# TinfoilHat0/Defending-Against-Backdoors-with-Robust-Learning-Rate

Hardware: NVIDIA H100
Metric: fl_rounds_per_sec (higher is better)
Workload: dtype bf16

## Files before the change

### defending-against-backdoors-with-robust-learning-rate_b200/ops/csrc/common.cuh

```cuda
#pragma once
#include <cuda_runtime.h>
#include <cuda_bf16.h>
#include <stdint.h>

#include "dropspec.h"
#include "kernels.h"

#define RLR_CUDA_CHECK(expr)                                                                     \
    do {                                                                                         \
        cudaError_t _e = (expr);                                                                 \
        if (_e != cudaSuccess) return _e;                                                        \
    } while (0)

namespace rlr {

constexpr int kWarp = 32;

__device__ __forceinline__ void pdl_wait() { asm volatile("griddepcontrol.wait;" ::: "memory"); }
__device__ __forceinline__ void pdl_trigger() { asm volatile("griddepcontrol.launch_dependents;" ::: "memory"); }

extern int g_pdl;
bool pdl_enabled();

template <typename... KArgs, typename... Args>
// ... 82 lines not shown
    auto stage = [&](int buf) {
#pragma unroll
        for (int q = 0; q < kPerThread; ++q) tile[buf][r0 + (256 / kCols) * q][c] = v[q];
    };
    load(0);
    stage(0);
    __syncthreads();
    T s = T(0);
    for (int k = 0; k < nchunks; ++k) {
        if (k + 1 < nchunks) load(k + 1);
        if (threadIdx.x < kCols) {
            const int rows = nparts - k * kRows < kRows ? nparts - k * kRows : kRows;
            int r = 0;
            if (k == 0) { s = tile[0][0][threadIdx.x]; r = 1; }
#pragma unroll 8
            for (; r < rows; ++r) s += tile[k & 1][r][threadIdx.x];
        }
        if (k + 1 < nchunks) stage((k + 1) & 1);
        __syncthreads();
    }
    if (threadIdx.x < kCols && col < n) out[col] += s;
}

__device__ __forceinline__ unsigned long long gtimer() {
    unsigned long long t;
    asm volatile("mov.u64 %0, %%globaltimer;" : "=l"(t));
    return t;
}

__device__ __forceinline__ float warp_sum(float v) {
#pragma unroll
    for (int o = 16; o > 0; o >>= 1) v += __shfl_xor_sync(0xffffffffu, v, o);
    return v;
}
__device__ __forceinline__ double warp_sum(double v) {
#pragma unroll
    for (int o = 16; o > 0; o >>= 1) v += __shfl_xor_sync(0xffffffffu, v, o);
    return v;
}
__device__ __forceinline__ unsigned long long warp_sum(unsigned long long v) {
#pragma unroll
    for (int o = 16; o > 0; o >>= 1) v += __shfl_xor_sync(0xffffffffu, v, o);
    return v;
}
__device__ __forceinline__ int warp_sum(int v) {
#pragma unroll
// ... 138 lines not shown
struct AugSpec {
    const long long* stream;
    unsigned long long seed;
    long long start;
    int pad, flip;
};
struct AugDraw { int oy, ox, flip; };
__device__ __forceinline__ AugDraw augment_draw(const AugSpec& a, long long pos) {
    const uint4 u = Philox(a.seed)((uint64_t)pos, (uint64_t)*a.stream);
    const uint32_t n = 2u * (uint32_t)a.pad + 1u;
    return {(int)(u.x % n), (int)(u.y % n), a.flip ? (int)(u.z & 1u) : 0};
}

__device__ __forceinline__ uint32_t dropout_keep8(const DropSpec& d, long long q) {
    const Philox ph(d.seed);
    const uint4 u = ph((uint64_t)q, ((uint64_t)(*d.step) << 20) ^ d.stream);
    const uint32_t r[4] = {u.x, u.y, u.z, u.w};
    uint32_t keep = 0;
#pragma unroll
    for (int i = 0; i < 8; ++i) keep |= (uint32_t)(((r[i >> 1] >> (16 * (i & 1))) & 0xffffu) >= d.thr) << i;
    return keep;
}

template <typename T>
inline cudaError_t launch_ordered_sum(T* out, const T* part, int nparts, long long n, cudaStream_t st) {
    if (nparts >= 16 && n <= 2048)
        return launch_kernel(ordered_sum_narrow_kernel<T>, dim3((unsigned)((n + 7) / 8)), dim3(256), (size_t)0, st, out, part, nparts, n);
    if (nparts >= 16)
        return launch_kernel(ordered_sum_cols_kernel<T>, dim3((unsigned)((n + 31) / 32)), dim3(256), (size_t)0, st, out, part, nparts, n);
    long long blocks = (n + 255) / 256;
    if (blocks > 1024) blocks = 1024;
    if (blocks < 1) blocks = 1;
    return launch_kernel(ordered_sum_kernel<T>, dim3((unsigned)blocks), dim3(256), (size_t)0, st, out, part, nparts, n);
}

__device__ __forceinline__ uint32_t pack_bf16x2(float lo, float hi) {
    __nv_bfloat162 v = __floats2bfloat162_rn(lo, hi);
    return *reinterpret_cast<uint32_t*>(&v);
}

}
```

### defending-against-backdoors-with-robust-learning-rate_b200/ops/csrc/gemm.h

```cpp
#pragma once
#include <cuda_runtime.h>
#include <cuda_bf16.h>
#include <stdint.h>

#include "dropspec.h"

namespace rlr {

constexpr int kStatSlots = 16;

struct ConvGemmParams {
    int M, N, num_kb;
    int mode;
    int cblocks;
    int TW, TH, TN;
    int Ho, Wo, NB;
    int tiles_w, tiles_h;
    int ntaps;
    int in_stride;
    int out_stride, out_ph, out_pw, OutH, OutW;
    int8_t dh[9], dw[9];
    int dn[9];
    int b_mn;
    int wtap[9];
// ... 27 lines not shown
void set_conv_occ3(int level);
void set_conv_one_wave(int on);
void set_conv_tma_store(int on);
void set_conv_split_producer(int on);
void set_conv_trace(long long* buf);
long long* conv_trace_buf();
cudaError_t launch_conv_bf16(const void* x, const void* w, void* out, int NB, int planes, int Hin, int Win, int Cin, int Ho, int Wo,
                             int Cout, int ldc, int ntaps, const int* dh, const int* dw, const int* dplane, const float* bias,
                             int relu, int accumulate, float* stats, cudaStream_t st, const int* wtap = nullptr, int w_taps_total = 0,
                             int in_stride = 1, int out_stride = 1, int out_ph = 0, int out_pw = 0);

cudaError_t launch_conv3x3_halo_bf16(const void* x, const void* w, void* out, int NB, int Hin, int Win, int H, int W, int Cout, const float* bias,
                                     int relu, int accumulate, float* stats, int bo_mode, long long* dbg, int num_sms, cudaStream_t st);

cudaError_t launch_conv3x3_halo3_bf16(const void* x, const void* w, void* out, int NB, int H, int W, int Cout, const float* bias, int relu,
                                      int accumulate, int num_sms, cudaStream_t st);

cudaError_t launch_conv_wgrad_bf16(const void* dy, const void* x, float* dW, int NB, int planes, int Hin, int Win, int Cin, int Cin_valid,
                                   int Ho, int Wo, int Cout, int ntaps, const int* dh, const int* dw, const int* dplane, int num_sms,
                                   cudaStream_t st, int in_stride = 1);
cudaError_t launch_conv_wgrad_halo_bf16(const void* dy, const void* x, float* dW, int NB, int H, int W, int Cin_valid, int Cout,
                                        int num_sms, cudaStream_t st);
cudaError_t launch_linear_wgrad_bf16(const void* dy, const void* x, float* dW, int B, int N, int K, int num_sms, cudaStream_t st);

cudaError_t launch_ordered_sum_f32(float* out, const float* part, int nparts, long long n, cudaStream_t st);
cudaError_t launch_ordered_sum_f64(double* out, const double* part, int nparts, long long n, cudaStream_t st);
cudaError_t launch_channel_stats(const __nv_bfloat16* x, long long M, int C, float* stats , int num_sms, cudaStream_t st,
                                 int only_sum = 0, int nslots = 1);
cudaError_t launch_bn_finalize(const float* stats, int slots, float* mean_rstd, float* running_mean, float* running_var, int C,
                               float count, float eps, float momentum, int train, cudaStream_t st);
cudaError_t launch_bn_apply(const __nv_bfloat16* x, const __nv_bfloat16* res, __nv_bfloat16* y, const float* gamma, const float* beta,
                            float* mean_rstd, long long M, int C, int relu, int fin_mode, const float* stats, int slots, float count,
                            float eps, float momentum, float* running_mean, float* running_var, int num_sms, cudaStream_t st);
cudaError_t launch_bn_bwd_reduce(const __nv_bfloat16* dy, const __nv_bfloat16* y, const __nv_bfloat16* x, const float* mean_rstd,
                                 float* dsum , long long M, int C, int relu, int num_sms, cudaStream_t st,
                                 const float* gamma = nullptr, const float* beta = nullptr, int nslots = 1);
cudaError_t launch_bn_bwd_apply(const __nv_bfloat16* dy, const __nv_bfloat16* y, const __nv_bfloat16* x, const float* gamma,
                                const float* mean_rstd, const float* dsum, __nv_bfloat16* dx, __nv_bfloat16* dres, float* dgamma,
                                float* dbeta, long long M, int C, int relu, int num_sms, cudaStream_t st, const float* beta = nullptr, int nslots = 1);
cudaError_t launch_gn_fwd(const __nv_bfloat16* x, const __nv_bfloat16* res, __nv_bfloat16* y, const float* gamma, const float* beta,
                          float* mean_rstd, int B, int HW, int C, int G, float eps, int relu, int num_sms, cudaStream_t st);
cudaError_t launch_gn_bwd(const __nv_bfloat16* dy, const __nv_bfloat16* y, const __nv_bfloat16* x, const float* gamma,
                          const float* mean_rstd, __nv_bfloat16* dx, __nv_bfloat16* dres, float* dgamma, float* dbeta, int B, int HW,
                          int C, int G, int relu, int num_sms, cudaStream_t st);
cudaError_t launch_relu_bwd(__nv_bfloat16* dy, const __nv_bfloat16* y, long long n, int num_sms, cudaStream_t st, float scale = 1.0f);
cudaError_t launch_maxpool2_fwd(const __nv_bfloat16* x, __nv_bfloat16* y, uint8_t* idx, int B, int H, int W, int C, cudaStream_t st,
                                float drop_p = 0.f, uint64_t seed = 0, const long long* step = nullptr, uint64_t stream = 0);
cudaError_t launch_maxpool2_bwd(const __nv_bfloat16* dy, const uint8_t* idx, __nv_bfloat16* dx, int B, int H, int W, int C, cudaStream_t st,
                                float drop_p, uint64_t seed, const long long* step, uint64_t stream, const __nv_bfloat16* zmask);
// ... 24 lines not shown
```

### defending-against-backdoors-with-robust-learning-rate_b200/ops/csrc/gemm_binding.cpp

```cpp
#include <torch/extension.h>
#include <ATen/cuda/CUDAContext.h>
#include <c10/cuda/CUDAGuard.h>
#include <c10/cuda/CUDAStream.h>
#include <c10/cuda/CUDACachingAllocator.h>

#include <vector>

#include "gemm.h"

namespace rlr {
void* scratch_alloc(size_t bytes, cudaStream_t st) {
    return c10::cuda::CUDACachingAllocator::raw_alloc_with_stream(bytes < 256 ? 256 : bytes, st);
}
void scratch_free(void* p) { c10::cuda::CUDACachingAllocator::raw_delete(p); }
}

namespace {
inline cudaStream_t cur_stream() { return c10::cuda::getCurrentCUDAStream().stream(); }
inline int num_sms() { return at::cuda::getCurrentDeviceProperties()->multiProcessorCount; }
inline void check(cudaError_t e, const char* what) { TORCH_CHECK(e == cudaSuccess, what, ": ", cudaGetErrorString(e)); }
template <typename T>
inline T* opt(const c10::optional<at::Tensor>& t) { return t.has_value() && t->defined() ? reinterpret_cast<T*>(t->data_ptr()) : nullptr; }
inline const __nv_bfloat16* bf(const at::Tensor& t) {
    TORCH_CHECK(t.is_cuda() && t.scalar_type() == at::kBFloat16 && t.is_contiguous(), "expected contiguous CUDA bf16 tensor");
// ... 124 lines not shown
    const int NB = x.size(0), Hin = x.size(1), Win = x.size(2), Cin = x.size(3), Ho = dy.size(1), Wo = dy.size(2), Cout = dy.size(3);
    const int T = (int)dh.size();
    TORCH_CHECK(dW.numel() == (int64_t)Cout * T * cin_valid);
    TORCH_CHECK((Cout <= 64 && Cout % 8 == 0) || Cout % 128 == 0, "wgrad: Cout must be <= 64 or a multiple of 128");
    int a[9], b[9], c[9] = {0};
    for (int t = 0; t < T; ++t) { a[t] = (int)dh[t]; b[t] = (int)dw[t]; }
    check(rlr::launch_conv_wgrad_bf16(bf(dy), bf(x), f32(dW), NB, 1, Hin, Win, Cin, (int)cin_valid, Ho, Wo, Cout, T, a, b, c, num_sms(),
                                      cur_stream(), (int)in_stride), "conv_wgrad_bf16_strided");
}
void conv_wgrad_halo_bf16(at::Tensor dy, at::Tensor x, at::Tensor dW, int64_t cin_valid) {
    c10::cuda::CUDAGuard g(x.device());
    TORCH_CHECK(x.dim() == 4 && x.size(3) == 64 && dy.dim() == 4 && dy.size(0) == x.size(0) && dy.size(1) == x.size(1) && dy.size(2) == x.size(2));
    TORCH_CHECK(dW.numel() == dy.size(3) * 9 * cin_valid);
    check(rlr::launch_conv_wgrad_halo_bf16(bf(dy), bf(x), f32(dW), x.size(0), x.size(1), x.size(2), (int)cin_valid, dy.size(3), num_sms(),
                                           cur_stream()), "conv_wgrad_halo_bf16");
}
void linear_wgrad_bf16(at::Tensor dy, at::Tensor x, at::Tensor dW) {
    c10::cuda::CUDAGuard g(x.device());
    const int B = x.size(0), K = x.size(1), N = dy.size(1);
    TORCH_CHECK(dy.size(0) == B && dW.numel() == (int64_t)N * K && ((N <= 64 && N % 8 == 0) || N % 128 == 0));
    check(rlr::launch_linear_wgrad_bf16(bf(dy), bf(x), f32(dW), B, N, K, num_sms(), cur_stream()), "linear_wgrad_bf16");
}

void ordered_sum(at::Tensor out, at::Tensor part) {
    c10::cuda::CUDAGuard g(out.device());
    TORCH_CHECK(out.is_contiguous() && part.is_contiguous() && part.dim() == 2 && part.size(1) == out.numel() &&
                part.scalar_type() == out.scalar_type(), "ordered_sum: out [n], part [nparts][n]");
    const int nparts = (int)part.size(0);
    const long long n = out.numel();
    if (out.scalar_type() == at::kDouble)
        check(rlr::launch_ordered_sum_f64(out.data_ptr<double>(), part.data_ptr<double>(), nparts, n, cur_stream()), "ordered_sum");
    else
        check(rlr::launch_ordered_sum_f32(out.data_ptr<float>(), part.data_ptr<float>(), nparts, n, cur_stream()), "ordered_sum");
}

void channel_stats(at::Tensor x, at::Tensor stats) {
    c10::cuda::CUDAGuard g(x.device());
    const int C = x.size(-1);
    const int nslots = (int)(stats.numel() / (2 * C));
    TORCH_CHECK(nslots >= 1 && stats.numel() == (int64_t)nslots * 2 * C, "stats must be [slots, 2, C]");
    check(rlr::launch_channel_stats(bf(x), x.numel() / C, C, f32(stats), num_sms(), cur_stream(), 0, nslots), "channel_stats");
}
void bias_grad(at::Tensor dy, at::Tensor db) {
    c10::cuda::CUDAGuard g(dy.device());
    const int C = dy.size(-1);
    TORCH_CHECK(db.numel() == C && db.scalar_type() == at::kFloat && dy.is_contiguous(), "bias_grad: db must be fp32 [C]");
    check(rlr::launch_channel_stats(bf(dy), dy.numel() / C, C, f32(db), num_sms(), cur_stream(), 1), "bias_grad");
}
void bn_finalize(at::Tensor stats, at::Tensor mean_rstd, at::Tensor rm, at::Tensor rv, double count, double eps, double momentum, bool train) {
    c10::cuda::CUDAGuard g(stats.device());
    const int C = mean_rstd.size(-1);
    const int slots = (int)(stats.numel() / (2 * C));
    TORCH_CHECK(slots >= 1 && stats.numel() == (int64_t)slots * 2 * C, "stats must be [slots, 2, C]");
    check(rlr::launch_bn_finalize(f32(stats), slots, f32(mean_rstd), (float*)rm.data_ptr(), (float*)rv.data_ptr(), C, (float)count, (float)eps,
                                  (float)momentum, train, cur_stream()), "bn_finalize");
}
// ... 134 lines not shown
                      bool accumulate_dx) {
    c10::cuda::CUDAGuard g(x.device());
    check(rlr::launch_linear_small_bwd(bf(x), bf(dy), bf(w), const_cast<__nv_bfloat16*>(bfo(dx)), (float*)dw.data_ptr(), opt<float>(db),
                                       x.size(0), x.size(1), w.size(0), accumulate_dx, cur_stream()), "linear_small_bwd");
}
void linear_small_fwd2(at::Tensor x, at::Tensor w, c10::optional<at::Tensor> bias, at::Tensor y, bool relu) {
    c10::cuda::CUDAGuard g(x.device());
    check(rlr::launch_linear_small_fwd2(bf(x), bf(w), opt<const float>(bias), bfm(y), x.size(0), x.size(1), w.size(0), relu, cur_stream()), "linear_small_fwd2");
}
void linear_small_bwd2(at::Tensor x, at::Tensor dy, at::Tensor w, c10::optional<at::Tensor> dx, at::Tensor dw, c10::optional<at::Tensor> db,
                       bool accumulate_dx) {
    c10::cuda::CUDAGuard g(x.device());
    check(rlr::launch_linear_small_bwd2(bf(x), bf(dy), bf(w), const_cast<__nv_bfloat16*>(bfo(dx)), (float*)dw.data_ptr(), opt<float>(db),
                                        x.size(0), x.size(1), w.size(0), accumulate_dx, cur_stream()), "linear_small_bwd2");
}
}

void register_gemm_bindings(py::module_& m) {
    m.attr("STAT_SLOTS") = rlr::kStatSlots;
    m.def("set_persistent_conv", [](bool on) { rlr::set_persistent_conv(on ? 1 : 0); });
    m.def("set_pdl", [](bool on) { rlr::set_pdl(on ? 1 : 0); });
    m.def("set_conv_occ3", [](int64_t level) { rlr::set_conv_occ3((int)level); });
    m.def("set_conv_one_wave", [](bool on) { rlr::set_conv_one_wave(on ? 1 : 0); });
    m.def("set_conv_tma_store", [](bool on) { rlr::set_conv_tma_store(on ? 1 : 0); });
    m.def("set_conv_split_producer", [](bool on) { rlr::set_conv_split_producer(on ? 1 : 0); });
    m.def("set_conv_trace", [](c10::optional<at::Tensor> buf) {
        rlr::set_conv_trace(buf.has_value() && buf->defined() ? reinterpret_cast<long long*>(buf->data_ptr<int64_t>()) : nullptr);
    });
    m.def("gemm_bf16", &gemm_bf16, py::arg("A"), py::arg("B"), py::arg("out"), py::arg("bias"), py::arg("relu"), py::arg("accumulate"), py::arg("stats"),
          py::arg("drop_p") = 0.0, py::arg("drop_seed") = 0, py::arg("drop_step") = py::none(), py::arg("drop_stream") = 0);
    m.def("stem_gemm_bf16", &stem_gemm_bf16, py::arg("A"), py::arg("W"), py::arg("out"), py::arg("bias"), py::arg("relu"), py::arg("stats"),
          py::arg("ready_ptr") = 0, py::arg("lo") = 0, py::arg("hi") = 0, py::arg("epoch") = py::none());
    m.def("gemm_splitk_bf16", &gemm_splitk_bf16, py::arg("A"), py::arg("B"), py::arg("out"), py::arg("ws"), py::arg("bias"), py::arg("relu"),
          py::arg("drop_p") = 0.0, py::arg("drop_seed") = 0, py::arg("drop_step") = py::none(), py::arg("drop_stream") = 0);
    m.def("conv_bf16", &conv_bf16);
    m.def("conv_bf16_strided", &conv_bf16_strided);
    m.def("conv_wgrad_bf16_strided", &conv_wgrad_bf16_strided);
    m.def("conv3x3_halo_bf16", &conv3x3_halo_bf16);
    m.def("conv3x3_halo3_bf16", &conv3x3_halo3_bf16);
    m.def("conv_wgrad_bf16", &conv_wgrad_bf16);
    m.def("linear_wgrad_bf16", &linear_wgrad_bf16);
    m.def("conv_wgrad_halo_bf16", &conv_wgrad_halo_bf16);
    m.def("channel_stats", &channel_stats);
    m.def("ordered_sum", &ordered_sum);
    m.def("bias_grad", &bias_grad);
    m.def("bn_finalize", &bn_finalize);
    m.def("bn_apply", &bn_apply);
    m.def("bn_bwd", &bn_bwd);
    m.def("bn_bwd_recompute", &bn_bwd_recompute);
    m.def("gn_fwd", &gn_fwd);
    m.def("gn_bwd", &gn_bwd);
    m.def("relu_bwd", &relu_bwd, py::arg("dy"), py::arg("y"), py::arg("scale") = 1.0);
    m.def("maxpool2_fwd", &maxpool2_fwd, py::arg("x"), py::arg("y"), py::arg("idx"), py::arg("drop_p") = 0.0, py::arg("drop_seed") = 0,
          py::arg("drop_step") = py::none(), py::arg("drop_stream") = 0);
    m.def("maxpool2_bwd", &maxpool2_bwd, py::arg("dy"), py::arg("idx"), py::arg("dx"), py::arg("drop_p") = 0.0, py::arg("drop_seed") = 0,
          py::arg("drop_step") = py::none(), py::arg("drop_stream") = 0, py::arg("relu_out") = py::none());
    m.def("avgpool_fwd", &avgpool_fwd);
    m.def("avgpool_bwd", &avgpool_bwd);
    m.def("dropout_fwd", &dropout_fwd);
    m.def("dropout_bwd", &dropout_bwd);
    m.def("space_to_depth", &space_to_depth);
    m.def("im2col_small", &im2col_small);
    m.def("filter_transpose", &filter_transpose);
    m.def("depth_to_space", &depth_to_space);
    m.def("filter_gather_transpose", &filter_gather_transpose);
    m.def("linear_small_fwd", &linear_small_fwd);
    m.def("linear_small_bwd", &linear_small_bwd);
// ... 4 lines not shown
```

### defending-against-backdoors-with-robust-learning-rate_b200/ops/csrc/norm.cu

```cuda
#include <stdlib.h>

#include "common.cuh"
#include "gemm.h"

namespace rlr {

struct bf8 { float v[8]; };
__device__ __forceinline__ bf8 unpack8(const uint4& u) {
    const __nv_bfloat162* h = reinterpret_cast<const __nv_bfloat162*>(&u);
    bf8 r;
#pragma unroll
    for (int i = 0; i < 4; ++i) { const float2 f = __bfloat1622float2(h[i]); r.v[2 * i] = f.x; r.v[2 * i + 1] = f.y; }
    return r;
}
__device__ __forceinline__ bf8 load8(const __nv_bfloat16* p) { return unpack8(*reinterpret_cast<const uint4*>(p)); }
__device__ __forceinline__ void store8(__nv_bfloat16* p, const bf8& r) {
    uint4 u;
    u.x = pack_bf16x2(r.v[0], r.v[1]); u.y = pack_bf16x2(r.v[2], r.v[3]);
    u.z = pack_bf16x2(r.v[4], r.v[5]); u.w = pack_bf16x2(r.v[6], r.v[7]);
    *reinterpret_cast<uint4*>(p) = u;
}
static inline int rows_grid(long long M, int rows_per_block, int num_sms, int per_sm) {
    long long want = (M + rows_per_block - 1) / rows_per_block;
    long long cap = (long long)num_sms * per_sm;
// ... 55 lines not shown
                    } else if (kRecompute) {
                        dz.x = (xv.x * msc[2 * i] + msh[2 * i]) > 0.f ? dz.x : 0.f;
                        dz.y = (xv.y * msc[2 * i + 1] + msh[2 * i + 1]) > 0.f ? dz.y : 0.f;
                    }
                    a[2 * i] += dz.x; a[2 * i + 1] += dz.y;
                    b[2 * i] += dz.x * (xv.x - mu[2 * i]) * rs[2 * i]; b[2 * i + 1] += dz.y * (xv.y - mu[2 * i + 1]) * rs[2 * i + 1];
                }
            }
        }
    }
    float* mine = sh + (size_t)ry * 2 * C + cg * 8;
#pragma unroll
    for (int i = 0; i < 8; ++i) { mine[i] = a[i]; mine[C + i] = b[i]; }
    __syncthreads();
    const int ncols = out_cols > 0 ? out_cols : 2 * C;
    float* dst = part + (size_t)blockIdx.x * ncols;
    for (int i = threadIdx.x; i < ncols; i += 256) {
        float t = 0.f;
        for (int r = 0; r < rpi; ++r) t += sh[(size_t)r * 2 * C + i];
        dst[i] = t;
    }
}

cudaError_t launch_ordered_sum_f32(float* out, const float* part, int nparts, long long n, cudaStream_t st) {
    return launch_ordered_sum(out, part, nparts, n, st);
}
cudaError_t launch_ordered_sum_f64(double* out, const double* part, int nparts, long long n, cudaStream_t st) {
    return launch_ordered_sum(out, part, nparts, n, st);
}

cudaError_t launch_channel_stats(const __nv_bfloat16* x, long long M, int C, float* stats, int num_sms, cudaStream_t st, int only_sum, int nslots) {
    if (!chan_ok(C) || nslots < 1) return cudaErrorInvalidValue;
    const int rpi = 256 / (C / 8);
    const int grid = rows_grid(M, rpi * 8, num_sms, nslots >= 4 ? 4 : 2), ncols = only_sum ? C : 2 * C;
    Scratch part((size_t)grid * ncols * sizeof(float), st);
    const size_t smem = (size_t)rpi * 2 * C * sizeof(float);
    auto kernel = nslots >= 4 ? channel_reduce_kernel<0, false, 4, 4> : channel_reduce_kernel<0, false, 8, 2>;
    RLR_CUDA_CHECK(launch_kernel(kernel, dim3(grid), dim3(256), smem, st, x, nullptr, nullptr, nullptr, part.as<float>(), M, C, 0, nullptr,
                                 nullptr, only_sum ? C : 0));
    return launch_ordered_sum(stats, part.as<float>(), grid, (long long)ncols, st);
}
cudaError_t launch_bn_bwd_reduce(const __nv_bfloat16* dy, const __nv_bfloat16* y, const __nv_bfloat16* x, const float* mean_rstd,
                                 float* dsum, long long M, int C, int relu, int num_sms, cudaStream_t st, const float* gamma,
                                 const float* beta, int nslots) {
    if (!chan_ok(C) || (relu == 2 && (!gamma || !beta)) || (relu == 1 && !y) || nslots < 1) return cudaErrorInvalidValue;
    const int rpi = 256 / (C / 8);
    const bool three = nslots >= 3;
    const int grid = rows_grid(M, rpi * 8, num_sms, three ? 3 : 2);
    const size_t smem = (size_t)rpi * 2 * C * sizeof(float);
    Scratch part((size_t)grid * 2 * C * sizeof(float), st);
    if (relu == 2)
// ... 750 lines not shown
```

### defending-against-backdoors-with-robust-learning-rate_b200/ops/csrc/wgrad.cu

```cuda
#include <cuda.h>
#include <stdlib.h>

#include "common.cuh"
#include "gemm.h"
#include "wgmma.cuh"

namespace rlr {

using namespace wg;

cudaError_t make_tmap_bf16(CUtensorMap* map, const void* base, int rank, const uint64_t* dims, const uint64_t* strides_bytes,
                           const uint32_t* box, const uint32_t* elem_strides = nullptr);

constexpr int WG_BM = 128, WG_BK = 64;
constexpr int WG_STAGES = 3;
constexpr int WG_A_BYTES = 2 * 64 * WG_BK * 2;
constexpr int WG_THREADS = 256 + 32;
template <int BNW>
struct WgCfg {
    static constexpr int kGroups = BNW / 64;
    static constexpr int kBBytes = kGroups * 64 * WG_BK * 2;
    static constexpr int kStageBytes = WG_A_BYTES + 3 * kBBytes;
    static constexpr int kSmem = WG_STAGES * kStageBytes + 2048;
};

struct WgradParams {
    int mode;
    int num_kb;
    int kb_per_cta;
    int a_groups;
    int ntaps_cta;
    int T;
    int TW, TH, TN, tiles_w, tiles_h;
    int8_t dh[9], dw[9];
    int dn[9];
    int in_stride;
    int ci_tiles;
    int Cout, Cin_valid;
    float* dW;
    float* part;
};

struct __align__(8) WgShared {
    uint64_t full[WG_STAGES];
    uint64_t empty[WG_STAGES];
};

template <int NACC, int BNW>
__device__ __forceinline__ void wgrad_flush(const float (&acc)[NACC / 2], float* dW, float* part, int co, int Cout, int T, int tap0, int ci0,
                                            int Cin_valid, int t) {
    if (part) dW = part + (size_t)blockIdx.z * Cout * T * Cin_valid;
#pragma unroll
    for (int h = 0; h < 2; ++h) {
        const int row = co + 8 * h;
        if (row >= Cout) continue;
#pragma unroll
        for (int j = 0; j < NACC / 8; ++j) {
            const int c = frag_col(t, 4 * j), tap = c / BNW, ci = ci0 + c % BNW;
            float* dst = dW + ((size_t)row * T + tap0 + tap) * Cin_valid + ci;
            const float a = acc[4 * j + 2 * h], b = acc[4 * j + 2 * h + 1];
            if (part) {
                if (ci < Cin_valid) dst[0] = a;
                if (ci + 1 < Cin_valid) dst[1] = b;
            } else if ((Cin_valid & 1) == 0) {
                if (ci < Cin_valid) asm volatile("red.global.add.v2.f32 [%0], {%1, %2};" ::"l"(dst), "f"(a), "f"(b) : "memory");
            } else {
                if (ci < Cin_valid) atomicAdd(dst, a);
                if (ci + 1 < Cin_valid) atomicAdd(dst + 1, b);
            }
        }
    }
}

template <int BNW, int kTaps>
__global__ void __launch_bounds__(WG_THREADS, 1)
umma_wgrad_kernel(const __grid_constant__ CUtensorMap tmA, const __grid_constant__ CUtensorMap tmB, const WgradParams p) {
    using Cfg = WgCfg<BNW>;
    constexpr int WG_BN = BNW, WG_B_BYTES = Cfg::kBBytes, WG_STAGE_BYTES = Cfg::kStageBytes;
    constexpr int NACC = kTaps * BNW;
    extern __shared__ uint8_t smem_raw[];
    uint8_t* smem = reinterpret_cast<uint8_t*>((reinterpret_cast<uintptr_t>(smem_raw) + 1023) & ~uintptr_t(1023));
    WgShared* sh = reinterpret_cast<WgShared*>(smem + WG_STAGES * WG_STAGE_BYTES);
    const int warp = threadIdx.x >> 5, lane = threadIdx.x & 31;
    const int co_tile = blockIdx.x / p.ci_tiles, ci_tile = blockIdx.x - co_tile * p.ci_tiles;
    const int tap0 = blockIdx.y * kTaps;
    const int kb_begin = blockIdx.z * p.kb_per_cta;
    const int kb_end = min(p.num_kb, kb_begin + p.kb_per_cta);
    const int nkb = kb_end - kb_begin;

    if (warp == 8 && lane == 0) {
        prefetch_tmap(&tmA); prefetch_tmap(&tmB);
        for (int s = 0; s < WG_STAGES; ++s) { mbar_init(&sh->full[s], 1); mbar_init(&sh->empty[s], 8); }
        fence_barrier_init();
    }
    __syncthreads();
    pdl_wait();
    pdl_trigger();

    if (warp == 8) {
        if (lane == 0) {
            int stage = 0;
            uint32_t phase = 0;
            const uint32_t bytes = p.a_groups * 8192 + kTaps * WG_B_BYTES;
            for (int i = 0; i < nkb; ++i) {
                const int kb = kb_begin + i;
                mbar_wait(&sh->empty[stage], phase ^ 1);
                uint8_t* sa = smem + stage * WG_STAGE_BYTES;
                uint8_t* sb = sa + WG_A_BYTES;
                mbar_expect_tx(&sh->full[stage], bytes);
                if (p.mode == 1) {
                    const int tw_i = kb % p.tiles_w, th_i = (kb / p.tiles_w) % p.tiles_h, tn_i = kb / (p.tiles_w * p.tiles_h);
                    const int w0 = tw_i * p.TW, h0 = th_i * p.TH, n0 = tn_i * p.TN;
                    for (int g = 0; g < p.a_groups; ++g)
                        tma_load_4d(&tmA, &sh->full[stage], sa + g * 8192, co_tile * WG_BM + g * 64, w0, h0, n0);
                    for (int t = 0; t < kTaps; ++t)
                        for (int g = 0; g < Cfg::kGroups; ++g)
                            tma_load_4d(&tmB, &sh->full[stage], sb + t * WG_B_BYTES + g * 8192, ci_tile * WG_BN + g * 64,
                                        w0 * p.in_stride + p.dw[tap0 + t], h0 * p.in_stride + p.dh[tap0 + t], n0 + p.dn[tap0 + t]);
                } else {
                    for (int g = 0; g < p.a_groups; ++g)
                        tma_load_2d(&tmA, &sh->full[stage], sa + g * 8192, co_tile * WG_BM + g * 64, kb * WG_BK);
                    for (int g = 0; g < Cfg::kGroups; ++g)
                        tma_load_2d(&tmB, &sh->full[stage], sb + g * 8192, ci_tile * WG_BN + g * 64, kb * WG_BK);
                }
                if (++stage == WG_STAGES) { stage = 0; phase ^= 1; }
            }
        }
    } else if (nkb > 0) {
        const int wgi = threadIdx.x >> 7, t = threadIdx.x & 127;
        const bool active = wgi < p.a_groups;
        float acc[NACC / 2];
#pragma unroll
        for (int i = 0; i < NACC / 2; ++i) acc[i] = 0.f;
        int stage = 0, prev = -1;
        uint32_t phase = 0;
        for (int i = 0; i < nkb; ++i) {
            mbar_wait(&sh->full[stage], phase);
            if (active) {
                const uint32_t sa = smem_u32(smem + stage * WG_STAGE_BYTES) + wgi * 8192;
                const uint32_t sb = smem_u32(smem + stage * WG_STAGE_BYTES) + WG_A_BYTES;
                wgmma_fence();
#pragma unroll
                for (int k = 0; k < WG_BK / 16; ++k) {
                    wgmma_bf16<NACC, 1, 1>(acc, smem_desc_sw128(sa + k * 2048, 8192, 1024), smem_desc_sw128(sb + k * 2048, 8192, 1024),
                                           (i > 0 || k > 0) ? 1u : 0u);
                }
                wgmma_commit();
                wgmma_wait<1>();
            }
            if (prev >= 0 && lane == 0) mbar_arrive(&sh->empty[prev]);
            prev = stage;
            if (++stage == WG_STAGES) { stage = 0; phase ^= 1; }
        }
        if (active) {
            wgmma_wait<0>();
            fence_acc(acc);
            wgrad_flush<NACC, BNW>(acc, p.dW, p.part, co_tile * WG_BM + wgi * 64 + frag_row(t, 0), p.Cout, p.T, tap0, ci_tile * WG_BN, p.Cin_valid, t);
        }
    }
}

template <int BNW, int kTaps>
static cudaError_t launch_wg(const CUtensorMap& tmA, const CUtensorMap& tmB, WgradParams& p, int co_tiles, int tap_groups,
                             int num_sms, cudaStream_t st) {
    static bool configured = false;
    if (!configured) {
        RLR_CUDA_CHECK(cudaFuncSetAttribute(umma_wgrad_kernel<BNW, kTaps>, cudaFuncAttributeMaxDynamicSharedMemorySize, WgCfg<BNW>::kSmem));
        configured = true;
    }
    const int base = co_tiles * p.ci_tiles * tap_groups;
    static const int tune_waves = [] { const char* e = getenv("RLR_WG_WAVES"); return e ? atoi(e) : 0; }();
    int waves = base >= num_sms ? (base + num_sms - 1) / num_sms : (tune_waves > 0 ? tune_waves : 1);
    int splits = (waves * num_sms) / base;
    if (splits > p.num_kb) splits = p.num_kb;
    if (splits < 1) splits = 1;
    p.kb_per_cta = (p.num_kb + splits - 1) / splits;
    splits = (p.num_kb + p.kb_per_cta - 1) / p.kb_per_cta;
    dim3 grid(co_tiles * p.ci_tiles, tap_groups, splits);
    if (splits == 1) return launch_kernel(umma_wgrad_kernel<BNW, kTaps>, grid, dim3(WG_THREADS), (size_t)WgCfg<BNW>::kSmem, st, tmA, tmB, p);
    const long long plane = (long long)p.Cout * p.T * p.Cin_valid;
    Scratch part((size_t)splits * plane * sizeof(float), st);
    p.part = part.as<float>();
    RLR_CUDA_CHECK(launch_kernel(umma_wgrad_kernel<BNW, kTaps>, grid, dim3(WG_THREADS), (size_t)WgCfg<BNW>::kSmem, st, tmA, tmB, p));
    return launch_ordered_sum(p.dW, p.part, splits, plane, st);
}

constexpr int WH_STAGES = 3;
constexpr int WH_A_BYTES = 2 * 128 * 128;
constexpr int WH_HALO_BYTES = 18 * 16 * 128;
constexpr int WH_STAGE_BYTES = WH_A_BYTES + WH_HALO_BYTES;
constexpr int WH_SMEM = WH_STAGES * WH_STAGE_BYTES + 2048;

struct WgHaloParams {
    int NB, H, W, tiles_h, tiles_w;
    int num_kb, kb_per_cta;
    int a_groups;
    int Cout, Cin_valid;
    float* dW;
    float* part;
};

__global__ void __launch_bounds__(WG_THREADS, 1)
umma_wgrad_halo_kernel(const __grid_constant__ CUtensorMap tmA, const __grid_constant__ CUtensorMap tmB, const WgHaloParams p) {
    extern __shared__ uint8_t smem_raw[];
    uint8_t* smem = reinterpret_cast<uint8_t*>((reinterpret_cast<uintptr_t>(smem_raw) + 1023) & ~uintptr_t(1023));
    WgShared* sh = reinterpret_cast<WgShared*>(smem + WH_STAGES * WH_STAGE_BYTES);
// ... 87 lines not shown
    splits = (p.num_kb + p.kb_per_cta - 1) / p.kb_per_cta;
    CUtensorMap tmA, tmB;
    {
        const uint64_t d[4] = {(uint64_t)Cout, (uint64_t)W, (uint64_t)H, (uint64_t)NB};
        const uint64_t s[3] = {(uint64_t)Cout * 2, (uint64_t)W * Cout * 2, (uint64_t)H * W * Cout * 2};
        const uint32_t b[4] = {64, 8, 16, 1};
        RLR_CUDA_CHECK(make_tmap_bf16(&tmA, dy, 4, d, s, b));
    }
    {
        const uint64_t d[4] = {64, (uint64_t)W, (uint64_t)H, (uint64_t)NB};
        const uint64_t s[3] = {128, (uint64_t)W * 128, (uint64_t)H * W * 128};
        const uint32_t b[4] = {64, 16, 18, 1};
        RLR_CUDA_CHECK(make_tmap_bf16(&tmB, x, 4, d, s, b));
    }
    if (splits == 1) return launch_kernel(umma_wgrad_halo_kernel, dim3(co_tiles, 3, splits), dim3(WG_THREADS), (size_t)WH_SMEM, st, tmA, tmB, p);
    const long long plane = (long long)Cout * 9 * Cin_valid;
    Scratch part((size_t)splits * plane * sizeof(float), st);
    p.part = part.as<float>();
    RLR_CUDA_CHECK(launch_kernel(umma_wgrad_halo_kernel, dim3(co_tiles, 3, splits), dim3(WG_THREADS), (size_t)WH_SMEM, st, tmA, tmB, p));
    return launch_ordered_sum(dW, p.part, splits, plane, st);
}

static int pow2_ceil_(int x) { int q = 1; while (q < x) q <<= 1; return q; }

cudaError_t launch_conv_wgrad_bf16(const void* dy, const void* x, float* dW, int NB, int planes, int Hin, int Win, int Cin, int Cin_valid,
                                   int Ho, int Wo, int Cout, int ntaps, const int* dh, const int* dw, const int* dplane, int num_sms,
                                   cudaStream_t st, int in_stride) {
    if (Cin % 64 || Cout % 8 || (ntaps != 1 && ntaps != 9)) return cudaErrorInvalidValue;
    if (in_stride < 1 || in_stride > 2 || (in_stride > 1 && planes != 1)) return cudaErrorInvalidValue;
    WgradParams p{};
    p.in_stride = in_stride;
    int TW = pow2_ceil_(Wo); if (TW > 64) TW = 64;
    int TH = pow2_ceil_(Ho); if (TW * TH > 64) TH = 64 / TW;
    const int TN = 64 / (TW * TH);
    p.mode = 1; p.TW = TW; p.TH = TH; p.TN = TN;
    p.tiles_w = (Wo + TW - 1) / TW; p.tiles_h = (Ho + TH - 1) / TH;
    p.num_kb = p.tiles_w * p.tiles_h * ((NB + TN - 1) / TN);
    p.T = ntaps; p.ntaps_cta = ntaps == 9 ? 3 : 1;
    for (int t = 0; t < ntaps; ++t) { p.dh[t] = (int8_t)dh[t]; p.dw[t] = (int8_t)dw[t]; p.dn[t] = dplane[t] * NB; }
    const bool wide = (Cin % 128 == 0) && (Cin_valid == Cin) && ntaps == 1;
    p.ci_tiles = wide ? Cin / 128 : Cin / 64; p.Cout = Cout; p.Cin_valid = Cin_valid; p.dW = dW;
    p.a_groups = Cout > 64 ? 2 : 1;
    const int co_tiles = (Cout + WG_BM - 1) / WG_BM;
    CUtensorMap tmA, tmB;
    {
        const uint64_t d[4] = {(uint64_t)Cout, (uint64_t)Wo, (uint64_t)Ho, (uint64_t)NB};
        const uint64_t s[3] = {(uint64_t)Cout * 2, (uint64_t)Wo * Cout * 2, (uint64_t)Ho * Wo * Cout * 2};
        const uint32_t b[4] = {64, (uint32_t)TW, (uint32_t)TH, (uint32_t)TN};
        RLR_CUDA_CHECK(make_tmap_bf16(&tmA, dy, 4, d, s, b));
    }
    {
        const uint64_t d[4] = {(uint64_t)Cin, (uint64_t)Win, (uint64_t)Hin, (uint64_t)planes * NB};
        const uint64_t s[3] = {(uint64_t)Cin * 2, (uint64_t)Win * Cin * 2, (uint64_t)Hin * Win * Cin * 2};
        const uint32_t b[4] = {64, (uint32_t)TW, (uint32_t)TH, (uint32_t)TN};
        const uint32_t es[4] = {1, (uint32_t)in_stride, (uint32_t)in_stride, 1};
        RLR_CUDA_CHECK(make_tmap_bf16(&tmB, x, 4, d, s, b, in_stride > 1 ? es : nullptr));
    }
    if (wide) return launch_wg<128, 1>(tmA, tmB, p, co_tiles, ntaps, num_sms, st);
    return ntaps == 9 ? launch_wg<64, 3>(tmA, tmB, p, co_tiles, 3, num_sms, st) : launch_wg<64, 1>(tmA, tmB, p, co_tiles, 1, num_sms, st);
}

cudaError_t launch_linear_wgrad_bf16(const void* dy, const void* x, float* dW, int B, int N, int K, int num_sms, cudaStream_t st) {
    if (N % 8 || K % 64) return cudaErrorInvalidValue;
    WgradParams p{};
    p.mode = 0; p.num_kb = (B + WG_BK - 1) / WG_BK; p.T = 1; p.ntaps_cta = 1; p.in_stride = 1;
    const bool wide = K % 128 == 0;
    p.ci_tiles = wide ? K / 128 : K / 64; p.Cout = N; p.Cin_valid = K; p.dW = dW;
    p.a_groups = N > 64 ? 2 : 1;
    const int co_tiles = (N + WG_BM - 1) / WG_BM;
    CUtensorMap tmA, tmB;
    {
        const uint64_t d[2] = {(uint64_t)N, (uint64_t)B}, s[1] = {(uint64_t)N * 2};
        const uint32_t b[2] = {64, WG_BK};
        RLR_CUDA_CHECK(make_tmap_bf16(&tmA, dy, 2, d, s, b));
    }
    {
        const uint64_t d[2] = {(uint64_t)K, (uint64_t)B}, s[1] = {(uint64_t)K * 2};
        const uint32_t b[2] = {64, WG_BK};
        RLR_CUDA_CHECK(make_tmap_bf16(&tmB, x, 2, d, s, b));
    }
    return wide ? launch_wg<128, 1>(tmA, tmB, p, co_tiles, 1, num_sms, st) : launch_wg<64, 1>(tmA, tmB, p, co_tiles, 1, num_sms, st);
// ... 4 lines not shown
```

Before: 0.6959.

## Load shared halo rows once per tap group in conv wgrad and deepen pipeline

Adds a halo-rows path for 3x3 conv weight-gradient: one TMA box covering the widened row tile is loaded per stage, and the three horizontally shifted taps read it through offset smem descriptors instead of three separate tile loads. Stage count now adapts to shared memory capacity (up to 8) rather than being fixed at 3. It also adds a vectorized wide ordered-sum kernel for few-part, many-column reductions of split-K partials. The risks are wgmma descriptor correctness when reading overlapping swizzled windows and extra template instantiations.

New measurement: 0.7093, median of 6. +1.9%, better.

```diff
diff --git a/defending-against-backdoors-with-robust-learning-rate_b200/ops/csrc/common.cuh b/defending-against-backdoors-with-robust-learning-rate_b200/ops/csrc/common.cuh
--- a/defending-against-backdoors-with-robust-learning-rate_b200/ops/csrc/common.cuh
+++ b/defending-against-backdoors-with-robust-learning-rate_b200/ops/csrc/common.cuh
@@ -128,6 +128,37 @@
     if (threadIdx.x < kCols && col < n) out[col] += s;
 }
 
+template <typename T, int V>
+struct alignas(sizeof(T) * V) SumVec { T v[V]; };
+template <typename T, int V>
+__global__ void __launch_bounds__(256) ordered_sum_wide_kernel(T* __restrict__ out, const T* __restrict__ part, int nparts, long long n) {
+    constexpr int kDepth = 8;
+    using Vec = SumVec<T, V>;
+    pdl_wait();
+    pdl_trigger();
+    const long long units = n / V;
+    for (long long u = (long long)blockIdx.x * 256 + threadIdx.x; u < units; u += (long long)gridDim.x * 256) {
+        const T* src = part + u * V;
+        Vec s = *reinterpret_cast<const Vec*>(src);
+        for (int j0 = 1; j0 < nparts; j0 += kDepth) {
+            Vec v[kDepth];
+#pragma unroll
+            for (int q = 0; q < kDepth; ++q)
+                if (j0 + q < nparts) v[q] = *reinterpret_cast<const Vec*>(src + (size_t)(j0 + q) * n);
+#pragma unroll
+            for (int q = 0; q < kDepth; ++q)
+                if (j0 + q < nparts) {
+#pragma unroll
+                    for (int e = 0; e < V; ++e) s.v[e] += v[q].v[e];
+                }
+        }
+        Vec o = *reinterpret_cast<const Vec*>(out + u * V);
+#pragma unroll
+        for (int e = 0; e < V; ++e) o.v[e] += s.v[e];
+        *reinterpret_cast<Vec*>(out + u * V) = o;
+    }
+}
+
 __device__ __forceinline__ unsigned long long gtimer() {
     unsigned long long t;
     asm volatile("mov.u64 %0, %%globaltimer;" : "=l"(t));
@@ -312,12 +343,31 @@
     return keep;
 }
 
-template <typename T>
-inline cudaError_t launch_ordered_sum(T* out, const T* part, int nparts, long long n, cudaStream_t st) {
-    if (nparts >= 16 && n <= 2048)
+enum OrderedSumKernel { kSumParts = 0, kSumCols = 1, kSumNarrow = 2, kSumWide = 3 };
+constexpr int kWideMaxParts = 16;
+constexpr long long kWideMinCols = 16384;
+inline int ordered_sum_kernel_for(int nparts, long long n) {
+    if (nparts <= kWideMaxParts && n >= kWideMinCols) return kSumWide;
+    if (nparts >= 16) return n <= 2048 ? kSumNarrow : kSumCols;
+    return kSumParts;
+}
+
+template <typename T>
+inline cudaError_t launch_ordered_sum(T* out, const T* part, int nparts, long long n, cudaStream_t st, int kernel = -1) {
+    if (kernel < 0) kernel = ordered_sum_kernel_for(nparts, n);
+    if (kernel == kSumNarrow)
         return launch_kernel(ordered_sum_narrow_kernel<T>, dim3((unsigned)((n + 7) / 8)), dim3(256), (size_t)0, st, out, part, nparts, n);
-    if (nparts >= 16)
+    if (kernel == kSumCols)
         return launch_kernel(ordered_sum_cols_kernel<T>, dim3((unsigned)((n + 31) / 32)), dim3(256), (size_t)0, st, out, part, nparts, n);
+    if (kernel == kSumWide) {
+        constexpr int V = 16 / sizeof(T);
+        const bool vec = n % V == 0 && ((reinterpret_cast<uintptr_t>(out) | reinterpret_cast<uintptr_t>(part)) & 15) == 0;
+        long long blocks = ((vec ? n / V : n) + 255) / 256;
+        if (blocks > 65535) blocks = 65535;
+        if (blocks < 1) blocks = 1;
+        return vec ? launch_kernel(ordered_sum_wide_kernel<T, V>, dim3((unsigned)blocks), dim3(256), (size_t)0, st, out, part, nparts, n)
+                   : launch_kernel(ordered_sum_wide_kernel<T, 1>, dim3((unsigned)blocks), dim3(256), (size_t)0, st, out, part, nparts, n);
+    }
     long long blocks = (n + 255) / 256;
     if (blocks > 1024) blocks = 1024;
     if (blocks < 1) blocks = 1;
diff --git a/defending-against-backdoors-with-robust-learning-rate_b200/ops/csrc/gemm.h b/defending-against-backdoors-with-robust-learning-rate_b200/ops/csrc/gemm.h
--- a/defending-against-backdoors-with-robust-learning-rate_b200/ops/csrc/gemm.h
+++ b/defending-against-backdoors-with-robust-learning-rate_b200/ops/csrc/gemm.h
@@ -73,9 +73,11 @@
 cudaError_t launch_conv_wgrad_halo_bf16(const void* dy, const void* x, float* dW, int NB, int H, int W, int Cin_valid, int Cout,
                                         int num_sms, cudaStream_t st);
 cudaError_t launch_linear_wgrad_bf16(const void* dy, const void* x, float* dW, int B, int N, int K, int num_sms, cudaStream_t st);
+void set_wgrad_halo_rows(int on);
+long long wgrad_halo_rows_launches();
 
-cudaError_t launch_ordered_sum_f32(float* out, const float* part, int nparts, long long n, cudaStream_t st);
-cudaError_t launch_ordered_sum_f64(double* out, const double* part, int nparts, long long n, cudaStream_t st);
+cudaError_t launch_ordered_sum_f32(float* out, const float* part, int nparts, long long n, cudaStream_t st, int kernel = -1);
+cudaError_t launch_ordered_sum_f64(double* out, const double* part, int nparts, long long n, cudaStream_t st, int kernel = -1);
 cudaError_t launch_channel_stats(const __nv_bfloat16* x, long long M, int C, float* stats , int num_sms, cudaStream_t st,
                                  int only_sum = 0, int nslots = 1);
 cudaError_t launch_bn_finalize(const float* stats, int slots, float* mean_rstd, float* running_mean, float* running_var, int C,
diff --git a/defending-against-backdoors-with-robust-learning-rate_b200/ops/csrc/gemm_binding.cpp b/defending-against-backdoors-with-robust-learning-rate_b200/ops/csrc/gemm_binding.cpp
--- a/defending-against-backdoors-with-robust-learning-rate_b200/ops/csrc/gemm_binding.cpp
+++ b/defending-against-backdoors-with-robust-learning-rate_b200/ops/csrc/gemm_binding.cpp
@@ -170,16 +170,17 @@
     check(rlr::launch_linear_wgrad_bf16(bf(dy), bf(x), f32(dW), B, N, K, num_sms(), cur_stream()), "linear_wgrad_bf16");
 }
 
-void ordered_sum(at::Tensor out, at::Tensor part) {
+void ordered_sum(at::Tensor out, at::Tensor part, int64_t kernel) {
     c10::cuda::CUDAGuard g(out.device());
     TORCH_CHECK(out.is_contiguous() && part.is_contiguous() && part.dim() == 2 && part.size(1) == out.numel() &&
                 part.scalar_type() == out.scalar_type(), "ordered_sum: out [n], part [nparts][n]");
+    TORCH_CHECK(kernel >= -1 && kernel <= 3, "ordered_sum: kernel must be -1 (rule) or 0..3");
     const int nparts = (int)part.size(0);
     const long long n = out.numel();
     if (out.scalar_type() == at::kDouble)
-        check(rlr::launch_ordered_sum_f64(out.data_ptr<double>(), part.data_ptr<double>(), nparts, n, cur_stream()), "ordered_sum");
+        check(rlr::launch_ordered_sum_f64(out.data_ptr<double>(), part.data_ptr<double>(), nparts, n, cur_stream(), (int)kernel), "ordered_sum");
     else
-        check(rlr::launch_ordered_sum_f32(out.data_ptr<float>(), part.data_ptr<float>(), nparts, n, cur_stream()), "ordered_sum");
+        check(rlr::launch_ordered_sum_f32(out.data_ptr<float>(), part.data_ptr<float>(), nparts, n, cur_stream(), (int)kernel), "ordered_sum");
 }
 
 void channel_stats(at::Tensor x, at::Tensor stats) {
@@ -360,6 +361,8 @@
     m.def("set_pdl", [](bool on) { rlr::set_pdl(on ? 1 : 0); });
     m.def("set_conv_occ3", [](int64_t level) { rlr::set_conv_occ3((int)level); });
     m.def("set_conv_one_wave", [](bool on) { rlr::set_conv_one_wave(on ? 1 : 0); });
+    m.def("set_wgrad_halo_rows", [](bool on) { rlr::set_wgrad_halo_rows(on ? 1 : 0); });
+    m.def("wgrad_halo_rows_launches", []() { return (int64_t)rlr::wgrad_halo_rows_launches(); });
     m.def("set_conv_tma_store", [](bool on) { rlr::set_conv_tma_store(on ? 1 : 0); });
     m.def("set_conv_split_producer", [](bool on) { rlr::set_conv_split_producer(on ? 1 : 0); });
     m.def("set_conv_trace", [](c10::optional<at::Tensor> buf) {
@@ -380,7 +383,7 @@
     m.def("linear_wgrad_bf16", &linear_wgrad_bf16);
     m.def("conv_wgrad_halo_bf16", &conv_wgrad_halo_bf16);
     m.def("channel_stats", &channel_stats);
-    m.def("ordered_sum", &ordered_sum);
+    m.def("ordered_sum", &ordered_sum, py::arg("out"), py::arg("part"), py::arg("kernel") = -1);
     m.def("bias_grad", &bias_grad);
     m.def("bn_finalize", &bn_finalize);
     m.def("bn_apply", &bn_apply);
diff --git a/defending-against-backdoors-with-robust-learning-rate_b200/ops/csrc/norm.cu b/defending-against-backdoors-with-robust-learning-rate_b200/ops/csrc/norm.cu
--- a/defending-against-backdoors-with-robust-learning-rate_b200/ops/csrc/norm.cu
+++ b/defending-against-backdoors-with-robust-learning-rate_b200/ops/csrc/norm.cu
@@ -101,11 +101,11 @@
     }
 }
 
-cudaError_t launch_ordered_sum_f32(float* out, const float* part, int nparts, long long n, cudaStream_t st) {
-    return launch_ordered_sum(out, part, nparts, n, st);
-}
-cudaError_t launch_ordered_sum_f64(double* out, const double* part, int nparts, long long n, cudaStream_t st) {
-    return launch_ordered_sum(out, part, nparts, n, st);
+cudaError_t launch_ordered_sum_f32(float* out, const float* part, int nparts, long long n, cudaStream_t st, int kernel) {
+    return launch_ordered_sum(out, part, nparts, n, st, kernel);
+}
+cudaError_t launch_ordered_sum_f64(double* out, const double* part, int nparts, long long n, cudaStream_t st, int kernel) {
+    return launch_ordered_sum(out, part, nparts, n, st, kernel);
 }
 
 cudaError_t launch_channel_stats(const __nv_bfloat16* x, long long M, int C, float* stats, int num_sms, cudaStream_t st, int only_sum, int nslots) {
diff --git a/defending-against-backdoors-with-robust-learning-rate_b200/ops/csrc/wgrad.cu b/defending-against-backdoors-with-robust-learning-rate_b200/ops/csrc/wgrad.cu
--- a/defending-against-backdoors-with-robust-learning-rate_b200/ops/csrc/wgrad.cu
+++ b/defending-against-backdoors-with-robust-learning-rate_b200/ops/csrc/wgrad.cu
@@ -13,15 +13,21 @@
                            const uint32_t* box, const uint32_t* elem_strides = nullptr);
 
 constexpr int WG_BM = 128, WG_BK = 64;
-constexpr int WG_STAGES = 3;
+constexpr int WG_HR_STAGES = 6;
+constexpr int WG_MAX_STAGES = 8;
+constexpr int WG_SMEM_LIMIT = 227 * 1024;
 constexpr int WG_A_BYTES = 2 * 64 * WG_BK * 2;
+constexpr int WG_HR_BYTES = 16 * 8 * 128;
 constexpr int WG_THREADS = 256 + 32;
-template <int BNW>
+template <int BNW, int kTaps, bool kHaloRows = false>
 struct WgCfg {
     static constexpr int kGroups = BNW / 64;
     static constexpr int kBBytes = kGroups * 64 * WG_BK * 2;
-    static constexpr int kStageBytes = WG_A_BYTES + 3 * kBBytes;
-    static constexpr int kSmem = WG_STAGES * kStageBytes + 2048;
+    static constexpr int kStageBytes = WG_A_BYTES + (kHaloRows ? WG_HR_BYTES : kTaps * kBBytes);
+    static constexpr int kFit = (WG_SMEM_LIMIT - 2048) / kStageBytes;
+    static constexpr int kStages = kHaloRows ? WG_HR_STAGES : (kFit < WG_MAX_STAGES ? kFit : WG_MAX_STAGES);
+    static constexpr int kSmem = kStages * kStageBytes + 2048;
+    static_assert(kStages <= WG_MAX_STAGES, "WgShared holds WG_MAX_STAGES barrier pairs");
 };
 
 struct WgradParams {
@@ -35,6 +41,8 @@
     int8_t dh[9], dw[9];
     int dn[9];
     int in_stride;
+    int hr_bytes;
+    int hr_kstep, hr_sbo;
     int ci_tiles;
     int Cout, Cin_valid;
     float* dW;
@@ -42,8 +50,8 @@
 };
 
 struct __align__(8) WgShared {
-    uint64_t full[WG_STAGES];
-    uint64_t empty[WG_STAGES];
+    uint64_t full[WG_MAX_STAGES];
+    uint64_t empty[WG_MAX_STAGES];
 };
 
 template <int NACC, int BNW>
@@ -72,15 +80,16 @@
     }
 }
 
-template <int BNW, int kTaps>
+template <int BNW, int kTaps, bool kHaloRows = false>
 __global__ void __launch_bounds__(WG_THREADS, 1)
 umma_wgrad_kernel(const __grid_constant__ CUtensorMap tmA, const __grid_constant__ CUtensorMap tmB, const WgradParams p) {
-    using Cfg = WgCfg<BNW>;
-    constexpr int WG_BN = BNW, WG_B_BYTES = Cfg::kBBytes, WG_STAGE_BYTES = Cfg::kStageBytes;
+    using Cfg = WgCfg<BNW, kTaps, kHaloRows>;
+    static_assert(!kHaloRows || (BNW == 64 && kTaps == 3), "halo rows: one 64-channel group, three taps");
+    constexpr int WG_BN = BNW, WG_B_BYTES = Cfg::kBBytes, WG_STAGE_BYTES = Cfg::kStageBytes, kStages = Cfg::kStages;
     constexpr int NACC = kTaps * BNW;
     extern __shared__ uint8_t smem_raw[];
     uint8_t* smem = reinterpret_cast<uint8_t*>((reinterpret_cast<uintptr_t>(smem_raw) + 1023) & ~uintptr_t(1023));
-    WgShared* sh = reinterpret_cast<WgShared*>(smem + WG_STAGES * WG_STAGE_BYTES);
+    WgShared* sh = reinterpret_cast<WgShared*>(smem + kStages * WG_STAGE_BYTES);
     const int warp = threadIdx.x >> 5, lane = threadIdx.x & 31;
     const int co_tile = blockIdx.x / p.ci_tiles, ci_tile = blockIdx.x - co_tile * p.ci_tiles;
     const int tap0 = blockIdx.y * kTaps;
@@ -90,7 +99,7 @@
 
     if (warp == 8 && lane == 0) {
         prefetch_tmap(&tmA); prefetch_tmap(&tmB);
-        for (int s = 0; s < WG_STAGES; ++s) { mbar_init(&sh->full[s], 1); mbar_init(&sh->empty[s], 8); }
+        for (int s = 0; s < kStages; ++s) { mbar_init(&sh->full[s], 1); mbar_init(&sh->empty[s], 8); }
         fence_barrier_init();
     }
     __syncthreads();
@@ -101,7 +110,7 @@
         if (lane == 0) {
             int stage = 0;
             uint32_t phase = 0;
-            const uint32_t bytes = p.a_groups * 8192 + kTaps * WG_B_BYTES;
+            const uint32_t bytes = p.a_groups * 8192 + (kHaloRows ? p.hr_bytes : kTaps * WG_B_BYTES);
             for (int i = 0; i < nkb; ++i) {
                 const int kb = kb_begin + i;
                 mbar_wait(&sh->empty[stage], phase ^ 1);
@@ -113,17 +122,20 @@
                     const int w0 = tw_i * p.TW, h0 = th_i * p.TH, n0 = tn_i * p.TN;
                     for (int g = 0; g < p.a_groups; ++g)
                         tma_load_4d(&tmA, &sh->full[stage], sa + g * 8192, co_tile * WG_BM + g * 64, w0, h0, n0);
-                    for (int t = 0; t < kTaps; ++t)
-                        for (int g = 0; g < Cfg::kGroups; ++g)
-                            tma_load_4d(&tmB, &sh->full[stage], sb + t * WG_B_BYTES + g * 8192, ci_tile * WG_BN + g * 64,
-                                        w0 * p.in_stride + p.dw[tap0 + t], h0 * p.in_stride + p.dh[tap0 + t], n0 + p.dn[tap0 + t]);
+                    if (kHaloRows)
+                        tma_load_4d(&tmB, &sh->full[stage], sb, ci_tile * WG_BN, w0 + p.dw[tap0], h0 + p.dh[tap0], n0 + p.dn[tap0]);
+                    else
+                        for (int t = 0; t < kTaps; ++t)
+                            for (int g = 0; g < Cfg::kGroups; ++g)
+                                tma_load_4d(&tmB, &sh->full[stage], sb + t * WG_B_BYTES + g * 8192, ci_tile * WG_BN + g * 64,
+                                            w0 * p.in_stride + p.dw[tap0 + t], h0 * p.in_stride + p.dh[tap0 + t], n0 + p.dn[tap0 + t]);
                 } else {
                     for (int g = 0; g < p.a_groups; ++g)
                         tma_load_2d(&tmA, &sh->full[stage], sa + g * 8192, co_tile * WG_BM + g * 64, kb * WG_BK);
                     for (int g = 0; g < Cfg::kGroups; ++g)
                         tma_load_2d(&tmB, &sh->full[stage], sb + g * 8192, ci_tile * WG_BN + g * 64, kb * WG_BK);
                 }
-                if (++stage == WG_STAGES) { stage = 0; phase ^= 1; }
+                if (++stage == kStages) { stage = 0; phase ^= 1; }
             }
         }
     } else if (nkb > 0) {
@@ -142,15 +154,15 @@
                 wgmma_fence();
 #pragma unroll
                 for (int k = 0; k < WG_BK / 16; ++k) {
-                    wgmma_bf16<NACC, 1, 1>(acc, smem_desc_sw128(sa + k * 2048, 8192, 1024), smem_desc_sw128(sb + k * 2048, 8192, 1024),
-                                           (i > 0 || k > 0) ? 1u : 0u);
+                    const uint64_t db = kHaloRows ? smem_desc_sw128(sb + k * p.hr_kstep, 128, p.hr_sbo) : smem_desc_sw128(sb + k * 2048, 8192, 1024);
+                    wgmma_bf16<NACC, 1, 1>(acc, smem_desc_sw128(sa + k * 2048, 8192, 1024), db, (i > 0 || k > 0) ? 1u : 0u);
                 }
                 wgmma_commit();
                 wgmma_wait<1>();
             }
             if (prev >= 0 && lane == 0) mbar_arrive(&sh->empty[prev]);
             prev = stage;
-            if (++stage == WG_STAGES) { stage = 0; phase ^= 1; }
+            if (++stage == kStages) { stage = 0; phase ^= 1; }
         }
         if (active) {
             wgmma_wait<0>();
@@ -160,12 +172,14 @@
     }
 }
 
-template <int BNW, int kTaps>
+template <int BNW, int kTaps, bool kHaloRows = false>
 static cudaError_t launch_wg(const CUtensorMap& tmA, const CUtensorMap& tmB, WgradParams& p, int co_tiles, int tap_groups,
                              int num_sms, cudaStream_t st) {
+    constexpr auto kernel = umma_wgrad_kernel<BNW, kTaps, kHaloRows>;
+    constexpr int kSmem = WgCfg<BNW, kTaps, kHaloRows>::kSmem;
     static bool configured = false;
     if (!configured) {
-        RLR_CUDA_CHECK(cudaFuncSetAttribute(umma_wgrad_kernel<BNW, kTaps>, cudaFuncAttributeMaxDynamicSharedMemorySize, WgCfg<BNW>::kSmem));
+        RLR_CUDA_CHECK(cudaFuncSetAttribute(kernel, cudaFuncAttributeMaxDynamicSharedMemorySize, kSmem));
         configured = true;
     }
     const int base = co_tiles * p.ci_tiles * tap_groups;
@@ -177,11 +191,11 @@
     p.kb_per_cta = (p.num_kb + splits - 1) / splits;
     splits = (p.num_kb + p.kb_per_cta - 1) / p.kb_per_cta;
     dim3 grid(co_tiles * p.ci_tiles, tap_groups, splits);
-    if (splits == 1) return launch_kernel(umma_wgrad_kernel<BNW, kTaps>, grid, dim3(WG_THREADS), (size_t)WgCfg<BNW>::kSmem, st, tmA, tmB, p);
+    if (splits == 1) return launch_kernel(kernel, grid, dim3(WG_THREADS), (size_t)kSmem, st, tmA, tmB, p);
     const long long plane = (long long)p.Cout * p.T * p.Cin_valid;
     Scratch part((size_t)splits * plane * sizeof(float), st);
     p.part = part.as<float>();
-    RLR_CUDA_CHECK(launch_kernel(umma_wgrad_kernel<BNW, kTaps>, grid, dim3(WG_THREADS), (size_t)WgCfg<BNW>::kSmem, st, tmA, tmB, p));
+    RLR_CUDA_CHECK(launch_kernel(kernel, grid, dim3(WG_THREADS), (size_t)kSmem, st, tmA, tmB, p));
     return launch_ordered_sum(p.dW, p.part, splits, plane, st);
 }
 
@@ -315,6 +329,20 @@
 }
 
 static int pow2_ceil_(int x) { int q = 1; while (q < x) q <<= 1; return q; }
+
+static int g_wgrad_halo_rows = 1;
+static long long g_wgrad_halo_rows_launches = 0;
+void set_wgrad_halo_rows(int on) { g_wgrad_halo_rows = on ? 1 : 0; }
+long long wgrad_halo_rows_launches() { return g_wgrad_halo_rows_launches; }
+
+static bool wgrad_halo_rows_ok(const WgradParams& p, int Wo, int planes, bool wide) {
+    if (!g_wgrad_halo_rows || wide || p.T != 9 || p.in_stride != 1 || planes != 1 || p.tiles_w != 1 || p.TN != 1) return false;
+    if (p.TW != Wo || (p.TW != 8 && p.TW != 16)) return false;
+    for (int r = 0; r < 3; ++r)
+        for (int t = 1; t < 3; ++t)
+            if (p.dh[3 * r + t] != p.dh[3 * r] || p.dw[3 * r + t] != p.dw[3 * r] + t || p.dn[3 * r + t] != p.dn[3 * r]) return false;
+    return true;
+}
 
 cudaError_t launch_conv_wgrad_bf16(const void* dy, const void* x, float* dW, int NB, int planes, int Hin, int Win, int Cin, int Cin_valid,
                                    int Ho, int Wo, int Cout, int ntaps, const int* dh, const int* dw, const int* dplane, int num_sms,
@@ -350,6 +378,18 @@
         RLR_CUDA_CHECK(make_tmap_bf16(&tmB, x, 4, d, s, b, in_stride > 1 ? es : nullptr));
     }
     if (wide) return launch_wg<128, 1>(tmA, tmB, p, co_tiles, ntaps, num_sms, st);
+    if (wgrad_halo_rows_ok(p, Wo, planes, wide)) {
+        const int Wh = TW == 16 ? 18 : 16;
+        p.hr_bytes = Wh * TH * 128;
+        p.hr_kstep = (16 / TW) * Wh * 128;
+        p.hr_sbo = TW == 16 ? 1024 : Wh * 128;
+        const uint64_t d[4] = {(uint64_t)Cin, (uint64_t)Win, (uint64_t)Hin, (uint64_t)NB};
+        const uint64_t s[3] = {(uint64_t)Cin * 2, (uint64_t)Win * Cin * 2, (uint64_t)Hin * Win * Cin * 2};
+        const uint32_t b[4] = {64, (uint32_t)Wh, (uint32_t)TH, 1};
+        RLR_CUDA_CHECK(make_tmap_bf16(&tmB, x, 4, d, s, b));
+        ++g_wgrad_halo_rows_launches;
+        return launch_wg<64, 3, true>(tmA, tmB, p, co_tiles, 3, num_sms, st);
+    }
     return ntaps == 9 ? launch_wg<64, 3>(tmA, tmB, p, co_tiles, 3, num_sms, st) : launch_wg<64, 1>(tmA, tmB, p, co_tiles, 1, num_sms, st);
 }
 
```
